# Yaling-Li/DMA-YOLO

Hardware: AMD Instinct MI355X
Metric: train images/sec (fwd+loss+bwd+optimizer, train.py batch loop) @1536; detect p50 ms incl. NMS (higher is better)
Workload: dtype bf16; 1 GPU; yolov5l-ca-sppfcspc-bifpn-scconv.yaml train @1536 nc=10; model=yolov5l-ca-sppfcspc-bifpn-scconv.yaml, global_batch=32, img=1536, parallelism=dp1

## Files before the change

### dma-yolo_amd/csrc/conv.hip

```cpp
#include <mutex>
#include "common.h"
#include <cstdlib>
#include <type_traits>
#include <atomic>
#include <cmath>

namespace {

constexpr int NT = 256;

template <typename T> struct Cfg;
template <> struct Cfg<bf16> {
  static constexpr int BK = 64, PADM = 8, PADK = 0;
};
template <> struct Cfg<float> {
  static constexpr int BK = 32, PADM = 4, PADK = 16;
};

template <typename T, int BM, int BN, bool AK, bool BKM> struct Tile {
  static constexpr int BK = Cfg<T>::BK, VW = Traits<T>::VW;
  static constexpr int RSM = BK + Cfg<T>::PADM;
  static constexpr int A_ELEMS = AK ? BK * (BM + Cfg<T>::PADK) : BM * RSM;
  static constexpr int B_ELEMS = BKM ? BK * (BN + Cfg<T>::PADK) : BN * RSM;
  static constexpr int STAGE = A_ELEMS + B_ELEMS;
// ... 65 lines not shown
    const int k = 4 * kk + (lane >> 4);
    float a[TM], b[TN];
#pragma unroll
    for (int i = 0; i < TM; ++i) {
      const int r = wm * (BM / 2) + i * 16 + (lane & 15);
      a[i] = AK ? As[kmaj_off<float, BM>(k, r)] : As[r * TT::RSM + k];
    }
#pragma unroll
    for (int j = 0; j < TN; ++j) {
      const int r = wn * (BN / 2) + j * 16 + (lane & 15);
      b[j] = BKM ? Bs[kmaj_off<float, BN>(k, r)] : Bs[r * TT::RSM + k];
    }
#pragma unroll
    for (int i = 0; i < TM; ++i)
#pragma unroll
      for (int j = 0; j < TN; ++j) acc[i][j] = __builtin_amdgcn_mfma_f32_16x16x4f32(a[i], b[j], acc[i][j], 0, 0, 0);
  }
}

template <typename T, int BM, int BN, bool AK, bool BKM, class L>
DEV void mainloop(L& ld, int kt0, int kt1, T* lds, f32x4 (&acc)[BM / 32][BN / 32]) {
  using TT = Tile<T, BM, BN, AK, BKM>;
  const int lane = threadIdx.x & 63, wid = threadIdx.x >> 6;
  const int wm = wid >> 1, wn = wid & 1;
  uint4 ra[L::CA], rb[L::CB];
  if (kt0 >= kt1) return;
  ld.load(kt0, ra, rb);
  int buf = 0;
  for (int kt = kt0; kt < kt1; ++kt) {
    T* As = lds + buf * TT::STAGE;
    T* Bs = As + TT::A_ELEMS;
    ld.store(As, Bs, ra, rb);
    __syncthreads();
    if (kt + 1 < kt1) ld.load(kt + 1, ra, rb);
    mma_step<BM, BN, AK, BKM>(As, Bs, acc, wm, wn, lane);
    buf ^= 1;
  }
}

template <typename T, int RSM> DEV void st_m(T* base, int row, int col, const uint4& v) {
  *reinterpret_cast<uint4*>(base + row * RSM + col) = v;
}
template <typename T, int ROW> DEV void st_k(T* base, int k, int row0, const uint4& v) {
  *reinterpret_cast<uint4*>(base + kmaj_off<T, ROW>(k, row0)) = v;
}

struct Geom {
  int N, H, W, C;
  int K, KH, KW, S, P;
  int OH, OW;
  long xps, yps;
  int oihw;
  int zeroed;
  float* dws;
  long dws_slab;
};

DEV void wgrad_out(const Geom& g, float* dw, int split, long idx, float v) {
  if (g.dws != nullptr) g.dws[(long)split * g.dws_slab + idx] = v;
  else atomicAdd(dw + idx, v);
}

struct Epi {
  const float* scale;
  const float* shift;
  const void* res;
  long rps;
  int act;
  int on;
};

DEV void epi_coef8(const Epi& ep, int n, float (&sc)[8], float (&sh)[8]) {
  const bool vs = (((uintptr_t)ep.scale | (uintptr_t)ep.shift) & 15) == 0;
#pragma unroll
  for (int h = 0; h < 2; ++h) {
    float4 a = make_float4(1.f, 1.f, 1.f, 1.f), b = make_float4(0.f, 0.f, 0.f, 0.f);
    if (vs) {
      if (ep.scale) a = *reinterpret_cast<const float4*>(ep.scale + n + 4 * h);
      if (ep.shift) b = *reinterpret_cast<const float4*>(ep.shift + n + 4 * h);
    } else {
      if (ep.scale) a = make_float4(ep.scale[n + 4 * h], ep.scale[n + 4 * h + 1], ep.scale[n + 4 * h + 2], ep.scale[n + 4 * h + 3]);
      if (ep.shift) b = make_float4(ep.shift[n + 4 * h], ep.shift[n + 4 * h + 1], ep.shift[n + 4 * h + 2], ep.shift[n + 4 * h + 3]);
    }
    sc[4 * h] = a.x; sc[4 * h + 1] = a.y; sc[4 * h + 2] = a.z; sc[4 * h + 3] = a.w;
    sh[4 * h] = b.x; sh[4 * h + 1] = b.y; sh[4 * h + 2] = b.z; sh[4 * h + 3] = b.w;
  }
}
DEV void epi_apply8(int act, float (&f)[8], const float (&sc)[8], const float (&sh)[8], const float* r) {
#pragma unroll
  for (int e = 0; e < 8; ++e) f[e] = f[e] * sc[e] + sh[e];
  act_fwd_n<8>(act, f);
  if (r != nullptr) {
#pragma unroll
    for (int e = 0; e < 8; ++e) f[e] += r[e];
  }
}

template <typename T, int VW>
DEV void epi_store(const Epi& ep, const T* src, T* dst, int n, int K, long m, bool full) {
  if constexpr (sizeof(T) == 2 && VW == 8) {
    if (full) {
      float f[8], sc[8], sh[8], r8[8];
      unpack<T>(*reinterpret_cast<const uint4*>(src), f);
      epi_coef8(ep, n, sc, sh);
      const T* rp = ep.res != nullptr ? reinterpret_cast<const T*>(ep.res) + m * ep.rps + n : nullptr;
      if (rp != nullptr) {
// ... 689 lines not shown
    }
  }
  DEV void issue(char* stage, int wid) {
    const bool kin = k < Ktot;
    const bf16* zero = reinterpret_cast<const bf16*>(g_zero_page);
#pragma unroll
    for (int j = 0; j < C3_::APW; ++j) {
      const bf16* src;
      if (P1) {
        src = (aval[j] && kin) ? x + abase[j] + k : zero;
      } else {
        const int ih = DG ? ih0[j] - kh : ih0[j] + kh, iw = DG ? iw0[j] - kw : iw0[j] + kw;
        const bool ok = aval[j] && kin && (unsigned)ih < (unsigned)g.H && (unsigned)iw < (unsigned)g.W;
        src = ok ? x + abase[j] + ((long)ih * g.W + iw) * g.xps + ci : zero;
      }
      glds16(src, stage + (wid * C3_::APW + j) * 1024);
    }
#pragma unroll
    for (int j = 0; j < C3_::BPW; ++j) {
      const bf16* src = (bval[j] && kin) ? w + boff[j] + k : zero;
      glds16(src, stage + C3_::A_BYTES + (wid * C3_::BPW + j) * 1024);
    }
    k += BK;
    if (!P1) {
      ci += BK;
      while (ci >= g.C) {
        ci -= g.C;
        if (++kw == g.KW) { kw = 0; ++kh; }
      }
    }
  }
};

constexpr unsigned kBufOob = 0xFFFFFFF0u;

DEV __amdgpu_buffer_rsrc_t make_rsrc(const void* base, unsigned bytes) {
  return __builtin_amdgcn_make_buffer_rsrc(const_cast<void*>(base), 0, (int)bytes, 0x00020000);
}
DEV void blds16(__amdgpu_buffer_rsrc_t r, unsigned off, char* lds_wave_base) {
  __builtin_amdgcn_raw_ptr_buffer_load_lds(r, (__attribute__((address_space(3))) void*)lds_wave_base, 16, off, 0, 0, 0);
}

struct S2Cls {
  int a, b, HX, WX;
};

template <int BM, int BN, int NS, bool P1, bool DG, bool S2 = false, int ES = 2, int WTR = 64>
struct FwdLdsB {
  using C3_ = Cfg3<BM, BN, NS, WTR>;
  static constexpr int BKE = 128 / ES;
  __amdgpu_buffer_rsrc_t rx, rw;
  int H, W, C, KW, xps;
  int kh, kw, ci0, kpos;
  int kw0, ca, cb, P;
  int kl;
  int pix[C3_::APW], ih0[C3_::APW], iw0[C3_::APW];
  bool aval[C3_::APW];
  unsigned boff[C3_::BPW];
  DEV FwdLdsB(const bf16* x, const bf16* w, const Geom& g, long M, long m0, int n0, int wid, int lane, unsigned xbytes,
              unsigned wbytes, S2Cls cls = S2Cls{0, 0, 0, 0})
      : H(g.H), W(g.W), C(g.C), KW(g.KW), xps((int)g.xps), kh(0), kw(0), ci0(0), kpos(0) {
    rx = make_rsrc(x, xbytes);
    rw = make_rsrc(w, wbytes);
    const int Ktot = g.KH * g.KW * g.C;
    P = g.P;
    ca = cls.a;
    cb = cls.b;
    kw0 = (cls.b + g.P) & 1;
    if (S2) { kh = (cls.a + g.P) & 1; kw = kw0; }
    kl = ((lane & 7) ^ ((lane >> 3) & 6)) * (16 / ES);
#pragma unroll
    for (int j = 0; j < C3_::APW; ++j) {
      const long m = m0 + apiece(wid, j) * 8 + (lane >> 3);
      aval[j] = m < M;
      const int mm = (int)(aval[j] ? m : 0);
      const int ow = mm % g.OW, t = mm / g.OW, oh = t % g.OH, b = t / g.OH;
      if (P1) { pix[j] = mm * xps; ih0[j] = 0; iw0[j] = 0; }
      else {
        ih0[j] = S2 ? oh : DG ? oh + g.P : oh * g.S - g.P;
        iw0[j] = S2 ? ow : DG ? ow + g.P : ow * g.S - g.P;
        pix[j] = ((b * g.H + ih0[j]) * g.W + iw0[j]) * xps;
      }
    }
#pragma unroll
    for (int j = 0; j < C3_::BPW; ++j) {
      const int n = n0 + (wid * C3_::BPW + j) * 8 + (lane >> 3);
      boff[j] = n < g.K ? (unsigned)(n * Ktot + kl) * (unsigned)ES : kBufOob;
    }
  }
  static DEV int apiece(int wid, int j) { return C3_::AEVEN ? wid * C3_::APW + j : j * C3_::NW + wid; }
  DEV void skip(int n) {
    kpos += n * BKE;
    if (!P1) {
      for (int i = 0; i < n; ++i) {
        ci0 += BKE;
        if (ci0 == C) {
          ci0 = 0;
          if (++kw == KW) {
            kw = 0;
            ++kh;
          }
        }
      }
    }
  }
  DEV void issue(char* stage, int wid) {
    const int dh = S2 ? (ca + P - kh) >> 1 : DG ? -kh : kh, dw = S2 ? (cb + P - kw) >> 1 : DG ? -kw : kw;
    const int delta = P1 ? kpos + kl : (dh * W + dw) * xps + ci0 + kl;
    const int bk = S2 ? (kh * KW + kw) * C + ci0 : kpos;
#pragma unroll
    for (int j = 0; j < C3_::APW; ++j) {
      const int pc = apiece(wid, j);
      if (!C3_::AEVEN && pc >= C3_::PA) break;
      bool ok = aval[j];
      if (!P1) ok = ok && (unsigned)(ih0[j] + dh) < (unsigned)H && (unsigned)(iw0[j] + dw) < (unsigned)W;
      blds16(rx, ok ? (unsigned)(pix[j] + delta) * (unsigned)ES : kBufOob, stage + pc * 1024);
    }
#pragma unroll
    for (int j = 0; j < C3_::BPW; ++j)
      blds16(rw, boff[j] == kBufOob ? kBufOob : boff[j] + (unsigned)bk * (unsigned)ES,
             stage + C3_::A_BYTES + (wid * C3_::BPW + j) * 1024);
    kpos += BKE;
    if (!P1) {
      ci0 += BKE;
      if (ci0 == C) {
        ci0 = 0;
        if (S2) {
          kw += 2;
          if (kw >= KW) { kw = kw0; kh += 2; }
        } else if (++kw == KW) {
          kw = 0;
          ++kh;
        }
      }
    }
  }
};

template <int N> DEV void vm_wait() { asm volatile("s_waitcnt vmcnt(%0)" ::"n"(N) : "memory"); }

template <int BM, int BN, int NS, class LD>
DEV void mainloop4(LD& ld, int nk, char* smem, f32x4 (&acc)[4][4], int wid, int lane) {
  using C3_ = Cfg3<BM, BN, NS>;
  constexpr int PER = C3_::APW + C3_::BPW;
  const int wm = wid % C3_::WM, wn = wid / C3_::WM;
  ld.issue(smem, wid);
  if (NS == 3 && nk > 1) ld.issue(smem + C3_::STAGE, wid);
  for (int kt = 0; kt < nk; ++kt) {
    if (NS == 3 && kt + 1 < nk) vm_wait<PER>();
    else vm_wait<0>();
    __builtin_amdgcn_s_barrier();
    const bf16* As = reinterpret_cast<const bf16*>(smem + (kt % NS) * C3_::STAGE);
    const bf16* Bs = As + BM * BK;
    bf16x8 a[2][4], b[2][4];
#pragma unroll
    for (int h = 0; h < 2; ++h) {
#pragma unroll
      for (int i = 0; i < 4; ++i) a[h][i] = frag_sw(As, wm * 64 + i * 16, h * 32, lane);
#pragma unroll
      for (int j = 0; j < 4; ++j) b[h][j] = frag_sw(Bs, wn * 64 + j * 16, h * 32, lane);
    }
    __builtin_amdgcn_sched_barrier(0);
    if (kt + NS - 1 < nk) ld.issue(smem + ((kt + NS - 1) % NS) * C3_::STAGE, wid);
    __builtin_amdgcn_sched_barrier(0);
#pragma unroll
    for (int h = 0; h < 2; ++h)
#pragma unroll
      for (int i = 0; i < 4; ++i)
#pragma unroll
        for (int j = 0; j < 4; ++j) acc[i][j] = __builtin_amdgcn_mfma_f32_16x16x32_bf16(a[h][i], b[h][j], acc[i][j], 0, 0, 0);
  }
}

template <int BM, int BN, int NS, class LD>
DEV void mainloop3(LD& ld, int nk, char* smem, f32x4 (&acc)[4][4], int wid, int lane) {
  using C3_ = Cfg3<BM, BN, NS>;
  constexpr int PER = C3_::APW + C3_::BPW;
  const int wm = wid % C3_::WM, wn = wid / C3_::WM;
  ld.issue(smem, wid);
  if (NS == 3 && nk > 1) ld.issue(smem + C3_::STAGE, wid);
  for (int kt = 0; kt < nk; ++kt) {
    if (NS == 3 && kt + 1 < nk) vm_wait<PER>();
    else vm_wait<0>();
    __builtin_amdgcn_s_barrier();
    if (kt + NS - 1 < nk) ld.issue(smem + ((kt + NS - 1) % NS) * C3_::STAGE, wid);
// ... 2010 lines not shown
          u4 o = {r0[0], r1[0], r0[1], r1[1]};
          if (accumulate) o = add_bf16x8(o, prev[i][j][gp >> 1]);
          if (EP) {
            const int n = 32 * j + 8 * gp + 8 * hf;
            float f[8], r8[8], sc[8], sh[8];
            unpack<bf16>(make_uint4(o[0], o[1], o[2], o[3]), f);
            if (resid) unpack<bf16>(make_uint4(prev[i][j][gp >> 1][0], prev[i][j][gp >> 1][1], prev[i][j][gp >> 1][2],
                                               prev[i][j][gp >> 1][3]), r8);
            const float4* cf = reinterpret_cast<const float4*>(smem + halo::LDS) + n / 4;
#pragma unroll
            for (int h = 0; h < 2; ++h) {
              const float4 a = cf[h], b = cf[16 + h];
              sc[4 * h] = a.x; sc[4 * h + 1] = a.y; sc[4 * h + 2] = a.z; sc[4 * h + 3] = a.w;
              sh[4 * h] = b.x; sh[4 * h + 1] = b.y; sh[4 * h + 2] = b.z; sh[4 * h + 3] = b.w;
            }
            epi_apply8(ep.act, f, sc, sh, resid ? r8 : nullptr);
            const uint4 q4 = pack<bf16>(f);
            o = u4{q4.x, q4.y, q4.z, q4.w};
          }
          const unsigned off = (mrow[i] + (unsigned)(32 * j + 8 * gp + 8 * hf)) * 2u;
          __builtin_amdgcn_raw_buffer_store_b128(o, ry, off, 0, 0);
        }
      }
    if (u + 1 < u1) vm_wait<8>();
  }
  if (!stats) return;
  vm_wait<0>();
  __syncthreads();
  float* red = reinterpret_cast<float*>(smem);
#pragma unroll
  for (int j = 0; j < 2; ++j)
#pragma unroll
    for (int r = 0; r < 16; ++r) {
      const int ch = 32 * j + (r & 3) + 8 * (r >> 2) + 4 * hf;
      red[(wid * 64 + ch) * 33 + px] = s1[j][r];
      red[((halo::NW + wid) * 64 + ch) * 33 + px] = s2[j][r];
    }
  __syncthreads();
  float t1 = 0.f, t2 = 0.f;
  for (int q = 0; q < 32; ++q) {
    t1 += red[(wid * 64 + lane) * 33 + q];
    t2 += red[((halo::NW + wid) * 64 + lane) * 33 + q];
  }
  const long row = (long)blockIdx.x * halo::NW + wid;
  psum[row * 64 + lane] = t1;
  psq[row * 64 + lane] = t2;
}
}

Geom make_geom(int N, int H, int W, int C, long xps, int K, int KH, int KW, int S, int P, int OH, int OW, long yps) {
  Geom g;
  g.N = N; g.H = H; g.W = W; g.C = C; g.K = K; g.KH = KH; g.KW = KW; g.S = S; g.P = P;
  g.OH = OH; g.OW = OW; g.xps = xps; g.yps = yps;
  g.oihw = 0; g.zeroed = 0;
  g.dws = nullptr; g.dws_slab = 0;
  return g;
}

__global__ void wgrad_split_reduce(const float* __restrict__ ws, float* __restrict__ dw, long slab, int splits) {
  for (long i = blockIdx.x * (long)blockDim.x + threadIdx.x; i < slab; i += (long)gridDim.x * blockDim.x) {
    float acc = ws[i];
    for (int k = 1; k < splits; ++k) acc += ws[(long)k * slab + i];
    dw[i] += acc;
  }
}

inline bool aligned16(const void* p) { return ((uintptr_t)p & 15) == 0; }
inline bool is_p1(const Geom& g) { return g.KH == 1 && g.KW == 1 && g.S == 1 && g.P == 0; }
inline double x_bytes(const Geom& g) { return 2.0 * ((double)g.N * g.H * g.W * g.xps); }
inline double y_bytes(const Geom& g) { return 2.0 * ((double)g.N * g.OH * g.OW * g.yps); }
inline double w_bytes(const Geom& g) { return 2.0 * g.K * g.KH * g.KW * g.C; }
inline bool fits_buf(double bytes) { return bytes < (double)v3::kBufOob; }

enum class Kern {
  HALO, SPLITK, P1S, STEM, P1P, PIPE8, WIDE, WIDE288, TALL, V3, V2,
  V2_BIG, S2_Q2S, S2_Q2, S2_MERGED, S2_CLASS,
  W_TAP128, W_TAP64, W_TAP64X2, W_V4, W_V3, W_V3N128, W_V3N256, W_V2_128, W_V2_64
};
struct Plan {
  Kern k;
  bool buf;
  bool lane;
  long rows;
};
struct WPlan {
  Kern k;
  int splits, per;
};

inline WPlan wgrad_split(Kern k, int tiles, int nk, double R, double t_step, double t_atomic) {
  int maxs = nk / 8;
  if (maxs < 1) maxs = 1;
  int splits = 1;
  double best = 1e300;
  for (int sp = 1; sp <= maxs; sp += (sp < 16 ? 1 : sp / 16)) {
    const double blocks = (double)tiles * sp;
    const double t = ceil(blocks / R) * ceil_div(nk, sp) * t_step + blocks * t_atomic;
    if (t < best) { best = t; splits = sp; }
  }
  const int per = ceil_div(nk, splits);
  return WPlan{k, ceil_div(nk, per), per};
}
inline WPlan wgrad_split_v2(Kern k, int tiles, int nk) {
  int splits = 2048 / tiles;
  if (splits < 1) splits = 1;
  int maxs = nk / 8;
  if (maxs < 1) maxs = 1;
  if (splits > maxs) splits = maxs;
  const int per = ceil_div(nk, splits);
  return WPlan{k, ceil_div(nk, per), per};
}

inline bool big_tile_rows(long M, int N) { return M >= 4096 && N > 64; }
inline bool big_tile(long M, int N) { return big_tile_rows(M, N) && ceil_div(M, 128) * ceil_div(N, 128) >= 256; }

template <typename T, int BM, int BN>
int launch_fwd(const T* x, const T* w, const float* b, T* y, float* ps, float* pq, const Geom& g, hipStream_t st,
               const Epi& ep = Epi{}) {
  constexpr int VW = Traits<T>::VW;
  const long M = (long)g.N * g.OH * g.OW;
  const int gm = ceil_div(M, BM), gn = ceil_div(g.K, BN);
  const bool p1 = is_p1(g);
  const bool vec = g.C % VW == 0 && g.xps % VW == 0 && aligned16(x);
  const unsigned grid = (unsigned)gm * gn;
  if (vec && p1) conv_fwd_kernel<T, BM, BN, true, true><<<grid, NT, 0, st>>>(x, w, b, y, ps, pq, g, gm, gn, ep);
  else if (vec) conv_fwd_kernel<T, BM, BN, true, false><<<grid, NT, 0, st>>>(x, w, b, y, ps, pq, g, gm, gn, ep);
  else if (p1) conv_fwd_kernel<T, BM, BN, false, true><<<grid, NT, 0, st>>>(x, w, b, y, ps, pq, g, gm, gn, ep);
  else conv_fwd_kernel<T, BM, BN, false, false><<<grid, NT, 0, st>>>(x, w, b, y, ps, pq, g, gm, gn, ep);
  return (int)hipGetLastError();
}

template <typename T, int BM, int BN>
int launch_dgrad(const T* dy, const T* wt, T* dx, int acc, const Geom& g, hipStream_t st) {
  constexpr int VW = Traits<T>::VW;
  const bool p1 = is_p1(g);
  const bool s2 = g.S == 2;
  const long M = s2 ? (long)g.N * ((g.H + 1) / 2) * ((g.W + 1) / 2) : (long)g.N * g.H * g.W;
// ... 144 lines not shown
      }
    }
    const int nprow = ps != nullptr ? dmy_conv_fwd_partial_rows(M, gv.K) : 0;
    v3::conv_p1p<BM, BN, NS, WTR, DG><<<(unsigned)G, PP::NTH, 0, st>>>(x, w, b, y, ps, pq, acc, gv, gm, gn, xbytes,
                                                                      wbytes, (unsigned)yb, nprow, ep, (unsigned)rb);
    return (int)hipGetLastError();
  });
}

inline long halo_units(const Geom& g) { return (long)g.N * (g.H / v3::halo::TH) * (g.W / v3::halo::TW); }
inline bool halo_ok(const Geom& g, const void* x, const void* w, const void* y) {
  if (g.KH != 3 || g.KW != 3 || g.S != 1 || g.P != 1 || g.C != 64 || g.K != 64 ||
      g.OH != g.H || g.OW != g.W || g.H % v3::halo::TH != 0 || g.W % v3::halo::TW != 0 || g.xps % 8 != 0 ||
      g.yps % 8 != 0 || !aligned16(x) || !aligned16(w) || !aligned16(y))
    return false;
  return fits_buf(x_bytes(g)) && fits_buf(y_bytes(g)) && halo_units(g) >= num_cus();
}
inline int halo_blocks(const Geom& g, int* per_out = nullptr) {
  const long nt = halo_units(g);
  const int per = ceil_div(nt, num_cus());
  if (per_out) *per_out = per;
  return ceil_div(nt, per);
}
inline int halo_rows(const Geom& g) { return v3::halo::NW * halo_blocks(g); }
template <bool DG>
int launch_halo(const bf16* x, const bf16* w, bf16* y, float* ps, float* pq, const Geom& g, hipStream_t st,
                int acc = 0, const Epi& ep = Epi{}) {
  const int thn = g.H / v3::halo::TH, twn = g.W / v3::halo::TW, nt = (int)halo_units(g);
  int per = 1;
  const int G = halo_blocks(g, &per);
  const unsigned xb = (unsigned)x_bytes(g), yb = (unsigned)y_bytes(g);
  const unsigned rb = ep.res != nullptr ? (unsigned)(2.0 * ((double)g.N * g.OH * g.OW * ep.rps)) : 0u;
  if (!DG && ep.on)
    v3::conv3_halo64<false, true><<<(unsigned)G, 64 * v3::halo::NW, 0, st>>>(x, w, y, ps, pq, g, twn, thn, nt, per,
                                                                           xb, 2u * 64 * 576, yb, acc, ep, rb);
  else
    v3::conv3_halo64<DG><<<(unsigned)G, 64 * v3::halo::NW, 0, st>>>(x, w, y, ps, pq, g, twn, thn, nt, per, xb,
                                                                    2u * 64 * 576, yb, acc, ep, rb);
  return (int)hipGetLastError();
}

template <bool DG>
Plan plan_v3(const Geom& gv, const void* x, const void* w, const void* y, int acc, const Epi& ep) {
  const long M = (long)gv.N * gv.OH * gv.OW;
  const bool p1 = is_p1(gv);
  Plan pl{Kern::V3, false, false, dmy_conv_fwd_partial_rows(M, gv.K)};
  if (DG && !ep.on && p1s_ok(gv, x, w, y) && gv.K >= 2 * gv.C && p1s_groups(gv.C, gv.K) <= 4)
    return pl.k = Kern::P1S, pl;
  if (!DG && !ep.on) {
    if (p1s_ok(gv, x, w, y) && gv.K >= 2 * gv.C) return pl.k = Kern::P1S, pl;
    if (stem_s_ok(gv, x, w, y)) return pl.k = Kern::STEM, pl;
  }
  pl.buf = gv.C % 64 == 0 && fits_buf(x_bytes(gv)) && fits_buf(w_bytes(gv));
  if (p1 && pl.buf && !ep.on && p1p_plan<DG>(gv, acc, ep, [](auto, auto, auto, auto) { return 0; }) >= 0) {
    pl.k = Kern::P1P;
    if (!DG) {
      const long r = p1p_lane_rows(gv);
      if (r > 0) pl.lane = true, pl.rows = r;
    }
    return pl;
  }
  if (pl.buf && gv.K >= kWideMinCols && (long)ceil_div(M, 256) * ceil_div(gv.K, 256) >= num_cus()) {
    if (p1 && ep.on && gv.C <= 128) return pl;
    if (p1) return pl.k = Kern::PIPE8, pl;
    if (wide_rows(M, ceil_div(gv.K, 256)) == 288) {
      pl.k = Kern::WIDE288;
      pl.rows = ceil_div(M, 288) * 2;
      return pl;
    }
    return pl.k = Kern::WIDE, pl;
  }
  if (pl.buf && !p1 && gv.K > 64 && gv.K <= 128 && (long)ceil_div(M, 512) * ceil_div(gv.K, 128) >= 4L * num_cus())
    return pl.k = Kern::TALL, pl;
  return pl;
}
template <bool DG>
int launch_v3(const bf16* x, const bf16* w, const float* b, bf16* y, float* ps, float* pq, int acc, const Geom& gv,
              hipStream_t st, const Epi& ep, const Plan& pl) {
  const long M = (long)gv.N * gv.OH * gv.OW;
  const bool p1 = is_p1(gv);
  const unsigned xbytes = pl.buf ? (unsigned)x_bytes(gv) : 0u, wbytes = pl.buf ? (unsigned)w_bytes(gv) : 0u;
#define W_GO(BM, BN)                                                                                                 \
  {                                                                                                                  \
    const int gm = ceil_div(M, BM), gn = ceil_div(gv.K, BN);                                                         \
    if (p1) v3::conv_fwd_w<BM, BN, true, DG><<<(unsigned)gm * gn, 512, 0, st>>>(x, w, b, y, ps, pq, acc, gv, gm, gn, \
                                                                              xbytes, wbytes, ep);                  \
    else v3::conv_fwd_w<BM, BN, false, DG><<<(unsigned)gm * gn, 512, 0, st>>>(x, w, b, y, ps, pq, acc, gv, gm, gn,   \
                                                                               xbytes, wbytes, ep);                 \
    return (int)hipGetLastError();                                                                                   \
  }
#define V3_GO(BM, BN, NS, BUF_)                                                                               \
  {                                                                                                           \
    const int gm = ceil_div(M, BM), gn = ceil_div(gv.K, BN);                                                  \
    if (p1)                                                                                                   \
      v3::conv_fwd_v3<BM, BN, NS, true, DG, BUF_><<<(unsigned)gm * gn, BM * BN / 64, 0, st>>>(                \
          x, w, b, y, ps, pq, acc, gv, gm, gn, xbytes, wbytes, v3::S2Cls{0, 0, 0, 0}, ep);                    \
    else                                                                                                      \
      v3::conv_fwd_v3<BM, BN, NS, false, DG, BUF_><<<(unsigned)gm * gn, BM * BN / 64, 0, st>>>(               \
          x, w, b, y, ps, pq, acc, gv, gm, gn, xbytes, wbytes, v3::S2Cls{0, 0, 0, 0}, ep);                    \
    return (int)hipGetLastError();                                                                            \
  }
  switch (pl.k) {
    case Kern::P1S: return launch_p1s<DG>(x, w, b, y, ps, pq, acc, gv, st);
    case Kern::STEM:
      return stem_nth(gv.K) == 512 ? launch_p1s_kd<160, 512, true>(x, w, b, y, ps, pq, acc, gv, st, 160, 1)
                                   : launch_p1s_kd<160, 768, true>(x, w, b, y, ps, pq, acc, gv, st, 160, 1);
    case Kern::P1P: return launch_p1p<DG>(x, w, b, y, ps, pq, acc, gv, st, xbytes, wbytes, ep, pl.lane);
    case Kern::PIPE8: {
      const int gm = ceil_div(M, 256), gn = ceil_div(gv.K, 256);
      v3::conv_fwd_8p<true, DG><<<(unsigned)gm * gn, 512, 0, st>>>(x, w, b, y, ps, pq, acc, gv, gm, gn, xbytes, wbytes, ep);
      return (int)hipGetLastError();
    }
    case Kern::WIDE: W_GO(256, 256)
    case Kern::WIDE288: W_GO(288, 256)
    case Kern::TALL: W_GO(512, 128)
    default: break;
  }
  if (gv.K > 64) {
    if (pl.buf) V3_GO(256, 128, 3, 1)
    V3_GO(256, 128, 3, 0)
  }
  if (pl.buf) V3_GO(256, 64, 2, 1)
  V3_GO(256, 64, 2, 0)
#undef W_GO
#undef V3_GO
}

__global__ void __launch_bounds__(256) splitk_epi_kernel(const float* __restrict__ ws, int splits, long M, int K,
                                                         const float* __restrict__ bias, bf16* __restrict__ y, long yps,
                                                         Epi ep) {
  const int CV = K / 8;
  const long total = M * CV;
  for (long v = blockIdx.x * 256L + threadIdx.x; v < total; v += (long)gridDim.x * 256) {
    const long m = v / CV;
    const int c = (int)(v - m * CV) * 8;
    float f[8];
#pragma unroll
    for (int j = 0; j < 8; ++j) f[j] = 0.f;
    for (int sp = 0; sp < splits; ++sp) {
      const float4* src = reinterpret_cast<const float4*>(ws + ((long)sp * M + m) * K + c);
      const float4 a = src[0], b = src[1];
      f[0] += a.x; f[1] += a.y; f[2] += a.z; f[3] += a.w;
      f[4] += b.x; f[5] += b.y; f[6] += b.z; f[7] += b.w;
    }
    bf16 t[8];
#pragma unroll
    for (int j = 0; j < 8; ++j) t[j] = __float2bfloat16(f[j] + (bias != nullptr ? bias[c + j] : 0.f));
    if (ep.on) epi_store<bf16, 8>(ep, t, y + m * yps + c, c, K, m, true);
    else *reinterpret_cast<uint4*>(y + m * yps + c) = *reinterpret_cast<const uint4*>(t);
  }
}

inline int splitk_plan(const Geom& g, const void* x, const void* w, const void* y, int& gm, int& gn, int& per) {
  const long M = (long)g.N * g.OH * g.OW;
  if (M >= 16384 || M == 0 || g.C % 64 != 0 || g.xps % 8 != 0 || g.K % 8 != 0 || g.yps % 8 != 0 || g.K < 32 ||
      !aligned16(x) || !aligned16(w) || !aligned16(y))
    return 0;
  if (!fits_buf(x_bytes(g)) || !fits_buf(w_bytes(g))) return 0;
  constexpr int pct = 200, mink = 2;
  if (g.KH == 1 && g.KW == 1) return 0;
  const int BN = g.K > 64 ? 128 : 64;
  gm = (int)ceil_div(M, 128);
  gn = ceil_div(g.K, BN);
  const int nk = g.KH * g.KW * g.C / v3::BK, tiles = gm * gn;
  int splits = ceil_div((long)pct * num_cus() / 100, tiles);
  if (splits > nk / mink) splits = nk / mink;
  if (splits < 2) return 0;
  per = ceil_div(nk, splits);
  return ceil_div(nk, per);
}

inline long splitk_elems(const Geom& g, const void* x, const void* w, const void* y) {
  int gm, gn, per;
  const int sp = splitk_plan(g, x, w, y, gm, gn, per);
  return sp ? (long)sp * g.N * g.OH * g.OW * g.K : 0;
}

inline int launch_splitk(const bf16* x, const bf16* w, const float* b, bf16* y, const Geom& g, float* ws, hipStream_t st,
                         const Epi& ep) {
  int gm, gn, per;
  const int sp = splitk_plan(g, x, w, y, gm, gn, per);
  const long M = (long)g.N * g.OH * g.OW;
  const unsigned xb = (unsigned)x_bytes(g), wb = (unsigned)w_bytes(g);
  const bool p1 = is_p1(g);
  const dim3 grid((unsigned)gm * gn, (unsigned)sp);
  if (g.K > 64) {
    if (p1) v3::conv_fwd_split<128, 128, 2, true><<<grid, 256, 0, st>>>(x, w, ws, g, gm, gn, per, xb, wb);
    else v3::conv_fwd_split<128, 128, 2, false><<<grid, 256, 0, st>>>(x, w, ws, g, gm, gn, per, xb, wb);
  } else {
    if (p1) v3::conv_fwd_split<128, 64, 2, true><<<grid, 128, 0, st>>>(x, w, ws, g, gm, gn, per, xb, wb);
    else v3::conv_fwd_split<128, 64, 2, false><<<grid, 128, 0, st>>>(x, w, ws, g, gm, gn, per, xb, wb);
  }
  splitk_epi_kernel<<<grid_cap(ceil_div(M * (g.K / 8), 256), 4096), 256, 0, st>>>(ws, sp, M, g.K, b, y, g.yps, ep);
  return (int)hipGetLastError();
}

Plan plan_fwd(const Geom& g, const void* x, const void* w, const float* b, const void* y, bool bn, const Epi& ep,
              long ws_elems) {
  const long M = (long)g.N * g.OH * g.OW;
  const bool res_ok = !ep.res || (ep.rps % 8 == 0 && aligned16(ep.res));
  if (b == nullptr && halo_ok(g, x, w, y) && (!ep.on || !bn) && halo_rows(g) <= prow_persist_cap() &&
      (!ep.on || ep.res == nullptr ||
       (res_ok && fits_buf(2.0 * ((double)g.N * g.OH * g.OW * ep.rps)))))
    return Plan{Kern::HALO, true, false, halo_rows(g)};
  if (ws_elems > 0 && !bn && res_ok) {
    const long need = splitk_elems(g, x, w, y);
    if (need > 0 && need <= ws_elems) return Plan{Kern::SPLITK, true, false, 0};
  }
  if (v3_ok(g.C, g.xps, g.K, g.yps, x, w, y, M) && res_ok) return plan_v3<false>(g, x, w, y, 0, ep);
  return Plan{Kern::V2, false, false, dmy_conv_fwd_partial_rows(M, g.K)};
}

template <typename T>
int conv_fwd_t(const void* x, const void* w, const float* b, void* y, float* ps, float* pq, const Geom& g, hipStream_t st,
               const Epi& ep = Epi{}, float* ws = nullptr, long ws_elems = 0) {
  const long M = (long)g.N * g.OH * g.OW;
  Plan pl{Kern::V2, false, false, dmy_conv_fwd_partial_rows(M, g.K)};
  if constexpr (sizeof(T) == 2) pl = plan_fwd(g, x, w, b, y, ps != nullptr, ep, ws != nullptr ? ws_elems : 0);
  if (ps != nullptr) t_prow_last = pl.rows;
  if constexpr (sizeof(T) == 2) {
    switch (pl.k) {
      case Kern::HALO: return launch_halo<false>((const bf16*)x, (const bf16*)w, (bf16*)y, ps, pq, g, st, 0, ep);
      case Kern::SPLITK: return launch_splitk((const bf16*)x, (const bf16*)w, b, (bf16*)y, g, ws, st, ep);
      case Kern::V2: break;
      default: return launch_v3<false>((const bf16*)x, (const bf16*)w, b, (bf16*)y, ps, pq, 0, g, st, ep, pl);
    }
  }
  if (ps != nullptr ? big_tile_rows(M, g.K) : big_tile(M, g.K))
    return launch_fwd<T, 128, 128>((const T*)x, (const T*)w, b, (T*)y, ps, pq, g, st, ep);
  return launch_fwd<T, 64, 64>((const T*)x, (const T*)w, b, (T*)y, ps, pq, g, st, ep);
}
inline Geom dgrad_view(const Geom& g) {
  return make_geom(g.N, g.OH, g.OW, g.K, g.yps, g.C, g.KH, g.KW, 1, g.P, g.H, g.W, g.xps);
}
inline Plan plan_dgrad_v2(const Geom& g) {
  const long M = (long)g.N * g.H * g.W / (g.S == 2 ? 4 : 1);
  return Plan{big_tile(M, g.C) ? Kern::V2_BIG : Kern::V2, false, false, 0};
}
Plan plan_dgrad(const Geom& g, const void* dy, const void* wt, const void* dx, int acc) {
  if (g.S == 2 && g.K % 64 == 0 && g.KH >= 2 && g.KW >= 2 &&
      v3_ok(g.K, g.yps, g.C, g.xps, dy, wt, dx, (long)g.N * (g.H / 2) * (g.W / 2)) && fits_buf(y_bytes(g)) &&
      fits_buf(w_bytes(g))) {
    Plan pl{Kern::S2_CLASS, true, false, 0};
    if ((g.C == 32 || g.C == 64 || g.C == 128) && g.KH == 3 && g.KW == 3 && g.P == 1 && g.OH == (g.H + 1) / 2 &&
        g.OW == (g.W + 1) / 2 && ceil_div((long)g.N * g.OH * g.OW, 256) >= num_cus())
      return pl.k = g.C == 32 ? Kern::S2_Q2S : Kern::S2_Q2, pl;
    if (g.C <= 64) return pl.k = Kern::S2_MERGED, pl;
    return pl;
  }
  const long M = (long)g.N * g.H * g.W;
  if (g.S == 1 && g.OH == g.H + 2 * g.P - g.KH + 1 && g.OW == g.W + 2 * g.P - g.KW + 1 &&
      v3_ok(g.K, g.yps, g.C, g.xps, dy, wt, dx, M)) {
    const Geom gv = dgrad_view(g);
    if (halo_ok(gv, dy, wt, dx)) return Plan{Kern::HALO, true, false, 0};
    return plan_v3<true>(gv, dy, wt, dx, acc, Epi{});
  }
  return plan_dgrad_v2(g);
}

inline int launch_dgrad_s2(const bf16* dy, const bf16* wt, bf16* dx, int acc, const Geom& g, hipStream_t st, Kern k) {
  const unsigned xbytes = (unsigned)y_bytes(g), wbytes = (unsigned)w_bytes(g);
  if (k == Kern::S2_Q2S || k == Kern::S2_Q2) {
    const int gm = (int)ceil_div((long)g.N * g.OH * g.OW, 256);
    const Geom gq = make_geom(g.N, g.OH, g.OW, g.K, g.yps, g.C == 32 ? 128 : 256, 2, 2, 1, 0, g.OH, g.OW, g.xps);
    const v3::S2Cls c0{0, 0, g.H, g.W};
    if (g.C == 32) v3::conv_dgrad_q2s<<<(unsigned)gm, 512, 0, st>>>(dy, wt, dx, acc, gq, gm, xbytes, wbytes, c0);
    else if (g.C == 64) v3::conv_dgrad_q2<64><<<(unsigned)gm, 512, 0, st>>>(dy, wt, dx, acc, gq, gm, xbytes, wbytes, c0);
    else v3::conv_dgrad_q2<128><<<(unsigned)(2 * gm), 512, 0, st>>>(dy, wt, dx, acc, gq, gm, xbytes, wbytes, c0);
    return (int)hipGetLastError();
  }
  if (k == Kern::S2_MERGED) {
    const long Mmax = (long)g.N * ((g.H + 1) / 2) * ((g.W + 1) / 2);
    const int gmax = ceil_div(Mmax, 256), gn = ceil_div(g.C, 64);
    v3::conv_dgrad_s2_v3<256, 64, 2><<<(unsigned)(4 * gmax * gn), 256, 0, st>>>(dy, wt, dx, acc, g, gmax, gn, xbytes,
                                                                              wbytes);
    return (int)hipGetLastError();
  }
  for (int a = 0; a < 2; ++a)
    for (int b = 0; b < 2; ++b) {
      const int H2 = (g.H - a + 1) / 2, W2 = (g.W - b + 1) / 2;
      if (H2 <= 0 || W2 <= 0) continue;
      const Geom gv = make_geom(g.N, g.OH, g.OW, g.K, g.yps, g.C, g.KH, g.KW, 2, g.P, H2, W2, g.xps);
      const long M = (long)g.N * H2 * W2;
      const v3::S2Cls cls{a, b, g.H, g.W};
      if (g.C % 256 == 0 && (long)ceil_div(M, 256) * (g.C / 256) >= num_cus()) {
        const int gn = g.C / 256;
        if (wide_rows(M, gn) == 288) {
          const int gm = ceil_div(M, 288);
          v3::conv_dgrad_s2_w<288, 256><<<(unsigned)gm * gn, 512, 0, st>>>(dy, wt, dx, acc, gv, gm, gn, xbytes, wbytes,
                                                                            cls);
        } else {
          const int gm = ceil_div(M, 256);
          v3::conv_dgrad_s2_w<256, 256><<<(unsigned)gm * gn, 512, 0, st>>>(dy, wt, dx, acc, gv, gm, gn, xbytes, wbytes,
                                                                            cls);
        }
      } else {
        const int gm = ceil_div(M, 256), gn = ceil_div(g.C, 128);
        v3::conv_fwd_v3<256, 128, 3, false, true, 3><<<(unsigned)gm * gn, 512, 0, st>>>(
            dy, wt, nullptr, dx, nullptr, nullptr, acc, gv, gm, gn, xbytes, wbytes, cls, Epi{});
      }
    }
  return (int)hipGetLastError();
}

template <typename T>
int conv_dgrad_t(const void* dy, const void* wt, void* dx, int acc, const Geom& g, hipStream_t st) {
  Plan pl = plan_dgrad_v2(g);
  if constexpr (sizeof(T) == 2) {
    pl = plan_dgrad(g, dy, wt, dx, acc);
    const bf16 *a = (const bf16*)dy, *b = (const bf16*)wt;
    switch (pl.k) {
      case Kern::V2:
      case Kern::V2_BIG: break;
      case Kern::S2_Q2S:
      case Kern::S2_Q2:
      case Kern::S2_MERGED:
      case Kern::S2_CLASS: return launch_dgrad_s2(a, b, (bf16*)dx, acc, g, st, pl.k);
      case Kern::HALO: return launch_halo<true>(a, b, (bf16*)dx, nullptr, nullptr, dgrad_view(g), st, acc);
      default: return launch_v3<true>(a, b, nullptr, (bf16*)dx, nullptr, nullptr, acc, dgrad_view(g), st, Epi{}, pl);
    }
  }
  if (pl.k == Kern::V2_BIG) return launch_dgrad<T, 128, 128>((const T*)dy, (const T*)wt, (T*)dx, acc, g, st);
  return launch_dgrad<T, 64, 64>((const T*)dy, (const T*)wt, (T*)dx, acc, g, st);
}
inline int num_cus() {
  static int n = [] {
    int dev = 0, v = 0;
    if (hipGetDevice(&dev) != hipSuccess || hipDeviceGetAttribute(&v, hipDeviceAttributeMultiprocessorCount, dev) != hipSuccess || v <= 0)
      v = 256;
    return v;
  }();
  return n;
}

inline bool wgrad_tap_ok(const Geom& g, const void* x, const void* dy) {
  if (g.KH != 3 || g.KW != 3 || g.S != 1 || g.P != 1 || g.OH != g.H || g.OW != g.W) return false;
  if (g.C % 16 != 0 || g.xps % 8 != 0 || g.yps % 8 != 0 || g.K % 8 != 0 || !aligned16(x) || !aligned16(dy)) return false;
  if (!fits_buf(x_bytes(g)) || !fits_buf(y_bytes(g))) return false;
  const long units = (long)g.N * ceil_div(g.OH, 8) * ceil_div(g.OW, 8) * ceil_div(g.K, 128) * ceil_div(g.C, 32);
  return units >= 10000;
}
inline int wgrad_narrow_for(const Geom& g, long NP) { return (g.K == 64 && NP >= 8L * 1024 * 1024) ? 1 : 2; }

template <typename T>
WPlan plan_wgrad(const Geom& g, const void* x, const void* dy) {
  const long NP = (long)g.N * g.OH * g.OW;
  const int Ntot = g.KH * g.KW * g.C;
  if constexpr (sizeof(T) == 2) {
    const bool vec = g.C % 8 == 0 && g.xps % 8 == 0 && g.K % 8 == 0 && g.yps % 8 == 0 && aligned16(x) && aligned16(dy);
    const int nm = wgrad_narrow_for(g, NP);
    const int nk = ceil_div(NP, 64);
    const double NC = num_cus();
    if (wgrad_tap_ok(g, x, dy)) {
      const Kern k = g.K > 64 ? Kern::W_TAP128 : g.C % 64 == 0 ? Kern::W_TAP64X2 : Kern::W_TAP64;
      const int BM = g.K > 64 ? 128 : 64, planes = k == Kern::W_TAP64X2 ? 2 : 1;
      const int np = g.N * ceil_div(g.OH, 8) * ceil_div(g.OW, 8);
      const double f = BM / 128.0 * planes;
      return wgrad_split(k, ceil_div(g.K, BM) * ceil_div(g.C, 32 * planes), np, 2.0 * NC, 1.1 * f, 0.113 * f);
    }
    if (vec && g.K >= 256 && Ntot >= 128 && NP >= 16384 && fits_buf(x_bytes(g)) && fits_buf(y_bytes(g)))
      return wgrad_split(Kern::W_V4, ceil_div(g.K, 256) * ceil_div(Ntot, 128), nk, NC, 1.9 * 2 * 0.5, 0.0504 * 2);
    if (vec && (g.K > 64 || nm == 2) && Ntot >= 64 && NP >= 16384)
      return wgrad_split(Kern::W_V3, ceil_div(g.K, 128) * ceil_div(Ntot, 128), nk, 2.0 * NC, 1.9, 0.0504);
    if (vec && g.K <= 64 && Ntot >= 128 && NP >= 16384 && nm == 1) {
      const bool wide = Ntot >= 512 || Ntot % 256 == 0 || (Ntot > 128 && Ntot < 256);
      const int BM = g.K <= 32 ? 32 : 64, BN = wide ? 256 : 128;
      const double R = 2.0 * NC * (128.0 * 128.0) / (BM * BN) * 0.5;
      const double step = 1.9 * (BM * BN) / (128.0 * 128.0) + 0.25;
      return wgrad_split(wide ? Kern::W_V3N256 : Kern::W_V3N128, ceil_div(g.K, BM) * ceil_div(Ntot, BN), nk, R, step,
                         0.0504 * (BM * BN) / (128.0 * 128.0));
// ... 171 lines not shown
  const Geom g = make_geom(N, H, W, C, xps, K, KH, KW, S, P, OH, OW, yps);
  if (!dtype) return dmy_conv_fwd_partial_rows((long)N * OH * OW, K);
  return (int)plan_fwd(g, x, w, bias, y, true, Epi{}, 0).rows;
}

DMY_API int dmy_conv_fwd(int dtype, const void* x, const void* w, const float* bias, void* y, float* psum, float* psq,
                         int N, int H, int W, int C, long xps, int K, int KH, int KW, int S, int P, int OH, int OW,
                         long yps, void* stream) {
  Geom g = make_geom(N, H, W, C, xps, K, KH, KW, S, P, OH, OW, yps);
  if ((long)N * OH * OW == 0 || K == 0) return 0;
  return dtype ? conv_fwd_t<bf16>(x, w, bias, y, psum, psq, g, (hipStream_t)stream)
               : conv_fwd_t<float>(x, w, bias, y, psum, psq, g, (hipStream_t)stream);
}

DMY_API int dmy_conv_fwd_act(int dtype, const void* x, const void* w, const float* bias, void* y, int N, int H, int W,
                             int C, long xps, int K, int KH, int KW, int S, int P, int OH, int OW, long yps,
                             const float* scale, const float* shift, int act, const void* res, long rps,
                             void* stream) {
  Geom g = make_geom(N, H, W, C, xps, K, KH, KW, S, P, OH, OW, yps);
  if ((long)N * OH * OW == 0 || K == 0) return 0;
  const Epi ep{scale, shift, res, rps, act, 1};
  return dtype ? conv_fwd_t<bf16>(x, w, bias, y, nullptr, nullptr, g, (hipStream_t)stream, ep)
               : conv_fwd_t<float>(x, w, bias, y, nullptr, nullptr, g, (hipStream_t)stream, ep);
}

DMY_API long dmy_fp8_quant_ws_elems() { return 1 + kF8Blocks; }
DMY_API int dmy_fp8_quant(const void* x, long rows, int C, long xps, void* x8, float* ws, void* stream) {
  if (C % 8 != 0 || xps % 8 != 0 || !aligned16(x) || rows * (C / 8) >= (1L << 31)) return (int)hipErrorInvalidValue;
  hipStream_t st = (hipStream_t)stream;
  const unsigned nvec = (unsigned)(rows * (C / 8));
  if (nvec == 0) {
    (void)hipMemsetAsync(ws, 0, sizeof(float), st);
    return (int)hipGetLastError();
  }
  const int grid = grid_cap(ceil_div(nvec, 256), kF8Blocks);
  fp8_blockmax_kernel<<<grid, 256, 0, st>>>((const bf16*)x, nvec, C / 8, xps, ws + 1);
  fp8_quant_kernel<<<grid, 256, 0, st>>>((const bf16*)x, nvec, C / 8, xps, (unsigned char*)x8, ws + 1, grid, ws);
  return (int)hipGetLastError();
}

DMY_API int dmy_conv_wprep_fp8(const float* w_oihw, void* w8, float* wscale, int K, int C, int KH, int KW,
                               void* stream) {
  if (C % 4 != 0) return (int)hipErrorInvalidValue;
  wprep_fp8_kernel<<<K, 256, 0, (hipStream_t)stream>>>(w_oihw, (unsigned char*)w8, wscale, C, KH, KW);
  return (int)hipGetLastError();
}

DMY_API int dmy_conv_fwd_fp8_partial_rows(long M, int K) { return 2 * ceil_div(M, K > 64 ? 128 : 64); }

DMY_API int dmy_conv_fwd_fp8(const void* x8, const void* w8, const float* xamax, const float* wscale,
                             const float* bias, void* y, float* psum, float* psq, int N, int H, int W, int C, int K,
                             int KH, int KW, int S, int P, int OH, int OW, long yps, const float* scale,
                             const float* shift, int act, const void* res, long rps, void* stream) {
  const Geom g = make_geom(N, H, W, C, C, K, KH, KW, S, P, OH, OW, yps);
  const long M = (long)N * OH * OW;
  if (M == 0 || K == 0) return 0;
  const double xb = (double)N * H * W * C, wb = (double)K * KH * KW * C;
  if (!fp8_fwd_ok(C, K, yps, x8, w8, y, xb, wb) || (res && (rps % 8 != 0 || !aligned16(res))))
    return (int)hipErrorInvalidValue;
  const Epi ep{scale, shift, res, rps, act, scale != nullptr || res != nullptr || act != 0 ? 1 : 0};
  const bool p1 = KH == 1 && KW == 1 && S == 1 && P == 0;
  hipStream_t st = (hipStream_t)stream;
  const unsigned xbytes = (unsigned)xb, wbytes = (unsigned)wb;
  const unsigned char *a = (const unsigned char*)x8, *b = (const unsigned char*)w8;
#define F8_GO(BM, BN, NS)                                                                                          \
  {                                                                                                                \
    const int gm = ceil_div(M, BM), gn = ceil_div(K, BN);                                                          \
    if (p1)                                                                                                        \
      v3::conv_fwd_f8<BM, BN, NS, true><<<(unsigned)gm * gn, BM * BN / 64, 0, st>>>(                                \
          a, b, xamax, wscale, bias, (bf16*)y, psum, psq, g, gm, gn, xbytes, wbytes, ep);                          \
    else                                                                                                           \
      v3::conv_fwd_f8<BM, BN, NS, false><<<(unsigned)gm * gn, BM * BN / 64, 0, st>>>(                               \
          a, b, xamax, wscale, bias, (bf16*)y, psum, psq, g, gm, gn, xbytes, wbytes, ep);                          \
  }
  if (K > 64) F8_GO(256, 128, 3)
  else F8_GO(256, 64, 2)
#undef F8_GO
  return (int)hipGetLastError();
}

DMY_API long dmy_conv_fwd_splitk_elems(int dtype, const void* x, const void* w, const void* y, int N, int H, int W,
                                       int C, long xps, int K, int KH, int KW, int S, int P, int OH, int OW, long yps) {
  if (!dtype) return 0;
  return splitk_elems(make_geom(N, H, W, C, xps, K, KH, KW, S, P, OH, OW, yps), x, w, y);
}

DMY_API int dmy_conv_fwd_act_ws(int dtype, const void* x, const void* w, const float* bias, void* y, int N, int H,
                                int W, int C, long xps, int K, int KH, int KW, int S, int P, int OH, int OW, long yps,
                                const float* scale, const float* shift, int act, const void* res, long rps, float* ws,
                                long ws_elems, void* stream) {
  Geom g = make_geom(N, H, W, C, xps, K, KH, KW, S, P, OH, OW, yps);
  if ((long)N * OH * OW == 0 || K == 0) return 0;
  const Epi ep{scale, shift, res, rps, act, scale != nullptr || res != nullptr || act != 0 ? 1 : 0};
  return dtype ? conv_fwd_t<bf16>(x, w, bias, y, nullptr, nullptr, g, (hipStream_t)stream, ep, ws, ws_elems)
               : conv_fwd_t<float>(x, w, bias, y, nullptr, nullptr, g, (hipStream_t)stream, ep);
}

DMY_API int dmy_conv_dgrad(int dtype, const void* dy, const void* wt, void* dx, int accumulate, int N, int H, int W,
                           int C, long xps, int K, int KH, int KW, int S, int P, int OH, int OW, long yps,
                           void* stream) {
  Geom g = make_geom(N, H, W, C, xps, K, KH, KW, S, P, OH, OW, yps);
  if ((long)N * H * W == 0 || C == 0) return 0;
  if (S > 2) return (int)hipErrorInvalidValue;
  return dtype ? conv_dgrad_t<bf16>(dy, wt, dx, accumulate, g, (hipStream_t)stream)
               : conv_dgrad_t<float>(dy, wt, dx, accumulate, g, (hipStream_t)stream);
}

// ... 95 lines not shown
```

Before: 163.4 images/s.

## Iterate conv K-loop with channel chunks outer and filter taps inner

Adds a channel-chunk-outer ordering of the reduction loop for the buffer-load implicit GEMM conv (forward, split-K, stride-2 dgrad, fp8). Successive k-steps now walk the filter taps for one channel chunk before moving to the next chunk, so neighbouring input tiles overlap spatially and hit cache more often. The skip() routine now computes tap and chunk directly instead of looping, and the weight offset is computed from (kh,kw,ci0) for all non-1x1 cases. The risk is that weight reads become strided across taps and that split-K partitioning changes which taps each split covers.

New measurement: 163.6 images/s, median of 6. Within noise of the previous version (+0.1%).

```diff
diff --git a/dma-yolo_amd/csrc/conv.hip b/dma-yolo_amd/csrc/conv.hip
--- a/dma-yolo_amd/csrc/conv.hip
+++ b/dma-yolo_amd/csrc/conv.hip
@@ -141,6 +141,7 @@
   long xps, yps;
   int oihw;
   int zeroed;
+  int kco;
   float* dws;
   long dws_slab;
 };
@@ -936,22 +937,25 @@
   __amdgpu_buffer_rsrc_t rx, rw;
   int H, W, C, KW, xps;
   int kh, kw, ci0, kpos;
-  int kw0, ca, cb, P;
+  int KH, kh0, kw0, ca, cb, P;
+  bool co;
   int kl;
   int pix[C3_::APW], ih0[C3_::APW], iw0[C3_::APW];
   bool aval[C3_::APW];
   unsigned boff[C3_::BPW];
   DEV FwdLdsB(const bf16* x, const bf16* w, const Geom& g, long M, long m0, int n0, int wid, int lane, unsigned xbytes,
               unsigned wbytes, S2Cls cls = S2Cls{0, 0, 0, 0})
-      : H(g.H), W(g.W), C(g.C), KW(g.KW), xps((int)g.xps), kh(0), kw(0), ci0(0), kpos(0) {
+      : H(g.H), W(g.W), C(g.C), KW(g.KW), xps((int)g.xps), ci0(0), kpos(0), KH(g.KH), co(g.kco != 0) {
     rx = make_rsrc(x, xbytes);
     rw = make_rsrc(w, wbytes);
     const int Ktot = g.KH * g.KW * g.C;
     P = g.P;
     ca = cls.a;
     cb = cls.b;
-    kw0 = (cls.b + g.P) & 1;
-    if (S2) { kh = (cls.a + g.P) & 1; kw = kw0; }
+    kh0 = S2 ? (cls.a + g.P) & 1 : 0;
+    kw0 = S2 ? (cls.b + g.P) & 1 : 0;
+    kh = kh0;
+    kw = kw0;
     kl = ((lane & 7) ^ ((lane >> 3) & 6)) * (16 / ES);
 #pragma unroll
     for (int j = 0; j < C3_::APW; ++j) {
@@ -973,25 +977,21 @@
     }
   }
   static DEV int apiece(int wid, int j) { return C3_::AEVEN ? wid * C3_::APW + j : j * C3_::NW + wid; }
+  static constexpr int TS = S2 ? 2 : 1;
   DEV void skip(int n) {
-    kpos += n * BKE;
+    kpos = n * BKE;
     if (!P1) {
-      for (int i = 0; i < n; ++i) {
-        ci0 += BKE;
-        if (ci0 == C) {
-          ci0 = 0;
-          if (++kw == KW) {
-            kw = 0;
-            ++kh;
-          }
-        }
-      }
+      const int ntw = (KW - kw0 + TS - 1) / TS, nth = (KH - kh0 + TS - 1) / TS, nc = C / BKE;
+      const int tap = co ? n % (nth * ntw) : n / nc, chunk = co ? n / (nth * ntw) : n % nc;
+      kh = kh0 + tap / ntw * TS;
+      kw = kw0 + tap % ntw * TS;
+      ci0 = chunk * BKE;
     }
   }
   DEV void issue(char* stage, int wid) {
     const int dh = S2 ? (ca + P - kh) >> 1 : DG ? -kh : kh, dw = S2 ? (cb + P - kw) >> 1 : DG ? -kw : kw;
     const int delta = P1 ? kpos + kl : (dh * W + dw) * xps + ci0 + kl;
-    const int bk = S2 ? (kh * KW + kw) * C + ci0 : kpos;
+    const int bk = P1 ? kpos : (kh * KW + kw) * C + ci0;
 #pragma unroll
     for (int j = 0; j < C3_::APW; ++j) {
       const int pc = apiece(wid, j);
@@ -1006,15 +1006,19 @@
              stage + C3_::A_BYTES + (wid * C3_::BPW + j) * 1024);
     kpos += BKE;
     if (!P1) {
-      ci0 += BKE;
-      if (ci0 == C) {
-        ci0 = 0;
-        if (S2) {
-          kw += 2;
-          if (kw >= KW) { kw = kw0; kh += 2; }
-        } else if (++kw == KW) {
-          kw = 0;
-          ++kh;
+      if (co) {
+        kw += TS;
+        if (kw >= KW) {
+          kw = kw0;
+          kh += TS;
+          if (kh >= KH) { kh = kh0; ci0 += BKE; }
+        }
+      } else {
+        ci0 += BKE;
+        if (ci0 == C) {
+          ci0 = 0;
+          kw += TS;
+          if (kw >= KW) { kw = kw0; kh += TS; }
         }
       }
     }
@@ -3131,7 +3135,7 @@
   Geom g;
   g.N = N; g.H = H; g.W = W; g.C = C; g.K = K; g.KH = KH; g.KW = KW; g.S = S; g.P = P;
   g.OH = OH; g.OW = OW; g.xps = xps; g.yps = yps;
-  g.oihw = 0; g.zeroed = 0;
+  g.oihw = 0; g.zeroed = 0; g.kco = 0;
   g.dws = nullptr; g.dws_slab = 0;
   return g;
 }
@@ -3161,7 +3165,9 @@
   bool buf;
   bool lane;
   long rows;
+  bool kco;
 };
+inline bool k_chunk_outer(const Geom& gv) { return gv.KH * gv.KW > 1; }
 struct WPlan {
   Kern k;
   int splits, per;
@@ -3412,6 +3418,7 @@
     if (stem_s_ok(gv, x, w, y)) return pl.k = Kern::STEM, pl;
   }
   pl.buf = gv.C % 64 == 0 && fits_buf(x_bytes(gv)) && fits_buf(w_bytes(gv));
+  pl.kco = pl.buf && k_chunk_outer(gv);
   if (p1 && pl.buf && !ep.on && p1p_plan<DG>(gv, acc, ep, [](auto, auto, auto, auto) { return 0; }) >= 0) {
     pl.k = Kern::P1P;
     if (!DG) {
@@ -3435,8 +3442,10 @@
   return pl;
 }
 template <bool DG>
-int launch_v3(const bf16* x, const bf16* w, const float* b, bf16* y, float* ps, float* pq, int acc, const Geom& gv,
+int launch_v3(const bf16* x, const bf16* w, const float* b, bf16* y, float* ps, float* pq, int acc, const Geom& gview,
               hipStream_t st, const Epi& ep, const Plan& pl) {
+  Geom gv = gview;
+  gv.kco = pl.kco;
   const long M = (long)gv.N * gv.OH * gv.OW;
   const bool p1 = is_p1(gv);
   const unsigned xbytes = pl.buf ? (unsigned)x_bytes(gv) : 0u, wbytes = pl.buf ? (unsigned)w_bytes(gv) : 0u;
@@ -3536,8 +3545,10 @@
   return sp ? (long)sp * g.N * g.OH * g.OW * g.K : 0;
 }
 
-inline int launch_splitk(const bf16* x, const bf16* w, const float* b, bf16* y, const Geom& g, float* ws, hipStream_t st,
-                         const Epi& ep) {
+inline int launch_splitk(const bf16* x, const bf16* w, const float* b, bf16* y, const Geom& gfwd, float* ws,
+                         hipStream_t st, const Epi& ep, const Plan& pl) {
+  Geom g = gfwd;
+  g.kco = pl.kco;
   int gm, gn, per;
   const int sp = splitk_plan(g, x, w, y, gm, gn, per);
   const long M = (long)g.N * g.OH * g.OW;
@@ -3565,7 +3576,7 @@
     return Plan{Kern::HALO, true, false, halo_rows(g)};
   if (ws_elems > 0 && !bn && res_ok) {
     const long need = splitk_elems(g, x, w, y);
-    if (need > 0 && need <= ws_elems) return Plan{Kern::SPLITK, true, false, 0};
+    if (need > 0 && need <= ws_elems) return Plan{Kern::SPLITK, true, false, 0, k_chunk_outer(g)};
   }
   if (v3_ok(g.C, g.xps, g.K, g.yps, x, w, y, M) && res_ok) return plan_v3<false>(g, x, w, y, 0, ep);
   return Plan{Kern::V2, false, false, dmy_conv_fwd_partial_rows(M, g.K)};
@@ -3581,7 +3592,7 @@
   if constexpr (sizeof(T) == 2) {
     switch (pl.k) {
       case Kern::HALO: return launch_halo<false>((const bf16*)x, (const bf16*)w, (bf16*)y, ps, pq, g, st, 0, ep);
-      case Kern::SPLITK: return launch_splitk((const bf16*)x, (const bf16*)w, b, (bf16*)y, g, ws, st, ep);
+      case Kern::SPLITK: return launch_splitk((const bf16*)x, (const bf16*)w, b, (bf16*)y, g, ws, st, ep, pl);
       case Kern::V2: break;
       default: return launch_v3<false>((const bf16*)x, (const bf16*)w, b, (bf16*)y, ps, pq, 0, g, st, ep, pl);
     }
@@ -3601,7 +3612,7 @@
   if (g.S == 2 && g.K % 64 == 0 && g.KH >= 2 && g.KW >= 2 &&
       v3_ok(g.K, g.yps, g.C, g.xps, dy, wt, dx, (long)g.N * (g.H / 2) * (g.W / 2)) && fits_buf(y_bytes(g)) &&
       fits_buf(w_bytes(g))) {
-    Plan pl{Kern::S2_CLASS, true, false, 0};
+    Plan pl{Kern::S2_CLASS, true, false, 0, true};
     if ((g.C == 32 || g.C == 64 || g.C == 128) && g.KH == 3 && g.KW == 3 && g.P == 1 && g.OH == (g.H + 1) / 2 &&
         g.OW == (g.W + 1) / 2 && ceil_div((long)g.N * g.OH * g.OW, 256) >= num_cus())
       return pl.k = g.C == 32 ? Kern::S2_Q2S : Kern::S2_Q2, pl;
@@ -3618,7 +3629,11 @@
   return plan_dgrad_v2(g);
 }
 
-inline int launch_dgrad_s2(const bf16* dy, const bf16* wt, bf16* dx, int acc, const Geom& g, hipStream_t st, Kern k) {
+inline int launch_dgrad_s2(const bf16* dy, const bf16* wt, bf16* dx, int acc, const Geom& gfwd, hipStream_t st,
+                           const Plan& pl) {
+  const Kern k = pl.k;
+  Geom g = gfwd;
+  g.kco = pl.kco;
   const unsigned xbytes = (unsigned)y_bytes(g), wbytes = (unsigned)w_bytes(g);
   if (k == Kern::S2_Q2S || k == Kern::S2_Q2) {
     const int gm = (int)ceil_div((long)g.N * g.OH * g.OW, 256);
@@ -3640,7 +3655,8 @@
     for (int b = 0; b < 2; ++b) {
       const int H2 = (g.H - a + 1) / 2, W2 = (g.W - b + 1) / 2;
       if (H2 <= 0 || W2 <= 0) continue;
-      const Geom gv = make_geom(g.N, g.OH, g.OW, g.K, g.yps, g.C, g.KH, g.KW, 2, g.P, H2, W2, g.xps);
+      Geom gv = make_geom(g.N, g.OH, g.OW, g.K, g.yps, g.C, g.KH, g.KW, 2, g.P, H2, W2, g.xps);
+      gv.kco = g.kco;
       const long M = (long)g.N * H2 * W2;
       const v3::S2Cls cls{a, b, g.H, g.W};
       if (g.C % 256 == 0 && (long)ceil_div(M, 256) * (g.C / 256) >= num_cus()) {
@@ -3675,7 +3691,7 @@
       case Kern::S2_Q2S:
       case Kern::S2_Q2:
       case Kern::S2_MERGED:
-      case Kern::S2_CLASS: return launch_dgrad_s2(a, b, (bf16*)dx, acc, g, st, pl.k);
+      case Kern::S2_CLASS: return launch_dgrad_s2(a, b, (bf16*)dx, acc, g, st, pl);
       case Kern::HALO: return launch_halo<true>(a, b, (bf16*)dx, nullptr, nullptr, dgrad_view(g), st, acc);
       default: return launch_v3<true>(a, b, nullptr, (bf16*)dx, nullptr, nullptr, acc, dgrad_view(g), st, Epi{}, pl);
     }
@@ -3953,7 +3969,8 @@
                              const float* bias, void* y, float* psum, float* psq, int N, int H, int W, int C, int K,
                              int KH, int KW, int S, int P, int OH, int OW, long yps, const float* scale,
                              const float* shift, int act, const void* res, long rps, void* stream) {
-  const Geom g = make_geom(N, H, W, C, C, K, KH, KW, S, P, OH, OW, yps);
+  Geom g = make_geom(N, H, W, C, C, K, KH, KW, S, P, OH, OW, yps);
+  g.kco = k_chunk_outer(g);
   const long M = (long)N * OH * OW;
   if (M == 0 || K == 0) return 0;
   const double xb = (double)N * H * W * C, wb = (double)K * KH * KW * C;
```
